# HeyWeCome/WhisprRec

Hardware: AMD Instinct MI355X
Metric: BPR training triplets/sec (higher is better)
Workload: dtype f32; 1 GPU; BPRMF emb_size=64, synthetic 1000000 users x 1000000 items (uniform ids), batch 65536, SGD l2=0, plan build in timed region; batch=65536, emb_size=64, optimizer=SGD, plan_chunk_batches=64, tables=single GPU, step_stream=whisprrec_amd.hip_ops.PipelinedSgd, plan=group plan (no per-batch sort: flags + lists of the shared rows, wr_group.hip), chained_step_launch=True, plan_build=on a side stream, beside the steps of the chunk before

## Files before the change

### whisprrec_amd/csrc/wr_group.hip

```cpp
#include "wr_common.h"
#include <hip/hip_ext.h>

#include <algorithm>

namespace wr {

constexpr int kGpThreads = 1024;
constexpr unsigned kGpRangeBits = 18;
constexpr int kGpWords = 1 << (kGpRangeBits - 5);
constexpr int kGpCap = 8192;
constexpr int kGpBins = 4096;
constexpr int kGpMaxBin = 256;
constexpr int kGpMaxRanges = 8;
constexpr int64_t kGpMaxBatch = 1 << 17;
constexpr int kGpLongRun = 64;
constexpr int kGpMetaWords = 16;
#ifndef WR_GP_DBG
#define WR_GP_DBG 0
#endif

struct GroupLayout {
    int64_t nb, B, fw;
    int R_u, R_i, cap_u, cap_i;
    unsigned mask_u, mask_i, hbits_u, hbits_i;
    int64_t flags, ucnt, icnt, ul_row, ul_src, il_row, il_src, total;
    int64_t zero_words;
};

static inline int ranges_for(int64_t n_rows, unsigned *mask, unsigned *hbits, int *cap) {
    unsigned bits = kGpRangeBits;
    while (bits < kGpRangeBits + 3 && (int64_t(1) << bits) < n_rows) ++bits;
    *mask = (1u << bits) - 1u;
    *hbits = bits;
    const int R = 1 << (bits - kGpRangeBits);
    *cap = kGpCap;
    return R;
}

static bool group_layout(int64_t n, int64_t B, int64_t n_users, int64_t n_items, GroupLayout &L) {
    if (n <= 0 || n >= (int64_t(1) << 31) || B <= 0 || B > kGpMaxBatch) return false;
    if (n_users <= 0 || n_users >= (int64_t(1) << 31) || n_items <= 0 || n_items >= (int64_t(1) << 31)) return false;
    L.nb = (n + B - 1) / B;
    L.B = B;
    L.fw = (B + 31) / 32;
    L.R_u = ranges_for(n_users, &L.mask_u, &L.hbits_u, &L.cap_u);
    L.R_i = ranges_for(n_items, &L.mask_i, &L.hbits_i, &L.cap_i);
    L.flags = kGpMetaWords;
    L.ucnt = L.flags + L.nb * L.fw * 4;
    L.icnt = L.ucnt + align_up(L.nb * L.R_u, 4);
    L.zero_words = L.icnt + align_up(L.nb * L.R_i, 4);
    L.ul_row = L.zero_words;
    L.ul_src = L.ul_row + L.nb * L.R_u * (int64_t)L.cap_u;
    L.il_row = L.ul_src + L.nb * L.R_u * (int64_t)L.cap_u;
    L.il_src = L.il_row + L.nb * L.R_i * (int64_t)L.cap_i;
    L.total = L.il_src + L.nb * L.R_i * (int64_t)L.cap_i;
    return true;
}

struct GpDev {
    int *meta;
    unsigned *flags;
    int *ucnt, *icnt;
    int *ul_row, *ul_src, *il_row, *il_src;
    int R_u, R_i, cap_u, cap_i;
    unsigned mask_u, mask_i, hbits_u, hbits_i;
    int fw;
};

static inline GpDev group_dev(int32_t *plan, const GroupLayout &L) {
    return GpDev{plan, reinterpret_cast<unsigned *>(plan + L.flags), plan + L.ucnt, plan + L.icnt, plan + L.ul_row,
                 plan + L.ul_src, plan + L.il_row, plan + L.il_src, L.R_u, L.R_i, L.cap_u, L.cap_i, L.mask_u, L.mask_i,
                 L.hbits_u, L.hbits_i, (int)L.fw};
}

template <typename F>
__device__ __forceinline__ void gp_scan(const int *__restrict__ a, int cnt, F f) {
    if ((reinterpret_cast<uintptr_t>(a) & 15u) == 0) {
        const int n4 = cnt >> 2;
        const int4 *a4 = reinterpret_cast<const int4 *>(a);
        int i = threadIdx.x;
        for (; i + 3 * kGpThreads < n4; i += 4 * kGpThreads) {
            int4 v[4];
#pragma unroll
            for (int q = 0; q < 4; ++q) v[q] = a4[i + q * kGpThreads];
#pragma unroll
            for (int q = 0; q < 4; ++q) {
                const int at = 4 * (i + q * kGpThreads);
                f(v[q].x, at);
                f(v[q].y, at + 1);
                f(v[q].z, at + 2);
                f(v[q].w, at + 3);
            }
        }
        for (; i < n4; i += kGpThreads) {
            const int4 v = a4[i];
            f(v.x, 4 * i);
            f(v.y, 4 * i + 1);
            f(v.z, 4 * i + 2);
            f(v.w, 4 * i + 3);
        }
        for (int j = (n4 << 2) + threadIdx.x; j < cnt; j += kGpThreads) f(a[j], j);
    } else {
        for (int j = threadIdx.x; j < cnt; j += kGpThreads) f(a[j], j);
    }
}

__global__ __launch_bounds__(kGpThreads) void group_plan_kernel(const int *__restrict__ u, const int *__restrict__ p,
                                                                 const int *__restrict__ n, int64_t n_total, int B, int nb,
                                                                 int n_users, int n_items, GpDev L) {
    extern __shared__ __attribute__((aligned(16))) unsigned gp_lds[];
    unsigned *seen = gp_lds;
    unsigned long long *keys = reinterpret_cast<unsigned long long *>(gp_lds);
    unsigned *multi = gp_lds + 2 * kGpCap;
    unsigned *f0 = multi + kGpWords, *f1 = f0 + L.fw, *f2 = f1 + L.fw;
    int &n_list = *reinterpret_cast<int *>(f2 + L.fw);
    const int per = L.R_u + L.R_i;
    const unsigned lb = xcd_contiguous_id(blockIdx.x, gridDim.x);
    const int b = (int)(lb / (unsigned)per), rr = (int)(lb % (unsigned)per);
    const bool item = rr >= L.R_u;
    const unsigned r = (unsigned)(item ? rr - L.R_u : rr);
    const int64_t base = (int64_t)b * B;
    const int Bb = (int)((base + B <= n_total) ? B : (n_total - base));
    const unsigned n_rows = (unsigned)(item ? n_items : n_users);
    const unsigned mask = item ? L.mask_i : L.mask_u;
    const unsigned rb = (item ? L.hbits_i : L.hbits_u) - kGpRangeBits, rsel = (1u << rb) - 1u;
    for (int i = threadIdx.x; i < kGpWords; i += kGpThreads) {
        seen[i] = 0u;
        multi[i] = 0u;
    }
    for (int i = threadIdx.x; i < 3 * L.fw; i += kGpThreads) f0[i] = 0u;
    if (threadIdx.x == 0) n_list = 0;
    __syncthreads();
    auto mark = [&](int row, int) {
        if ((unsigned)row >= n_rows) {
            L.meta[0] = 1;
            return;
        }
        const unsigned h = (unsigned)row & mask;
        if ((h & rsel) != r) return;
        const unsigned bit = h >> rb, m = 1u << (bit & 31u);
        const unsigned old = atomicOr(&seen[bit >> 5], m);
        if (old & m) atomicOr(&multi[bit >> 5], m);
    };
    if (!(WR_GP_DBG & 8)) {
        if (item) {
            gp_scan(p + base, Bb, mark);
            gp_scan(n + base, Bb, mark);
        } else {
            gp_scan(u + base, Bb, mark);
        }
    }
    __syncthreads();
    auto several = [&](int row) -> bool {
        const unsigned h = (unsigned)row & mask;
        if ((h & rsel) != r) return false;
        const unsigned bit = h >> rb;
        return (multi[bit >> 5] >> (bit & 31u)) & 1u;
    };
    auto append = [&](int row, unsigned src) {
        const int pos = atomicAdd(&n_list, 1);
        if (pos < kGpCap) keys[pos] = ((unsigned long long)(unsigned)row << 32) | src;
    };
    if (!(WR_GP_DBG & 2)) {
        const bool next = b + 1 < nb && !(WR_GP_DBG & 16);
        const int64_t nbase = base + B;
        const int Bn = next ? (int)((nbase + B <= n_total) ? B : (n_total - nbase)) : 0;
        auto defer = [&](int row, int t) {
            if (several(row)) atomicOr(&f2[t >> 5], 1u << (t & 31));
        };
        if (item) {
            gp_scan(p + base, Bb, [&](int row, int t) {
                if (several(row)) {
                    atomicOr(&f0[t >> 5], 1u << (t & 31));
                    append(row, (unsigned)t << 1);
                }
            });
            gp_scan(n + base, Bb, [&](int row, int t) {
                if (several(row)) {
                    atomicOr(&f1[t >> 5], 1u << (t & 31));
                    append(row, ((unsigned)t << 1) | 1u);
                }
            });
            gp_scan(p + nbase, Bn, defer);
            gp_scan(n + nbase, Bn, defer);
        } else {
            gp_scan(u + base, Bb, [&](int row, int t) {
                if (several(row)) {
                    atomicOr(&f0[t >> 5], 1u << (t & 31));
                    append(row, (unsigned)t << 1);
                }
            });
            gp_scan(u + nbase, Bn, defer);
        }
    }
    __syncthreads();
    if (!(WR_GP_DBG & 4)) {
        unsigned *fb = L.flags + (int64_t)b * L.fw * 4;
        for (int w = threadIdx.x; w < L.fw; w += kGpThreads) {
            if (f0[w]) __hip_atomic_fetch_or(fb + 4 * w + (item ? 1 : 0), f0[w], __ATOMIC_RELAXED, __HIP_MEMORY_SCOPE_AGENT);
            if (item && f1[w]) __hip_atomic_fetch_or(fb + 4 * w + 2, f1[w], __ATOMIC_RELAXED, __HIP_MEMORY_SCOPE_AGENT);
            if (f2[w])
                __hip_atomic_fetch_or(fb + 4 * (L.fw + w) + 3, f2[w], __ATOMIC_RELAXED, __HIP_MEMORY_SCOPE_AGENT);
        }
    }
    const int cap = item ? L.cap_i : L.cap_u, R = item ? L.R_i : L.R_u;
    int m = n_list;
    if (m > cap) {
        if (threadIdx.x == 0) L.meta[1] = 1;
        m = cap;
    }
    int *cnt = reinterpret_cast<int *>(multi);
    unsigned short *out16 = reinterpret_cast<unsigned short *>(multi + kGpBins);
    int *wave_tot = reinterpret_cast<int *>(f0);
    auto bin_of = [&](unsigned long long k) -> int { return (int)(((((unsigned)(k >> 32)) & mask) >> rb) & (kGpBins - 1)); };
    int *lrow = (item ? L.il_row : L.ul_row) + ((int64_t)b * R + r) * cap, *lsrc = (item ? L.il_src : L.ul_src) + ((int64_t)b * R + r) * cap;
    __syncthreads();
    for (int i = threadIdx.x; i < kGpBins; i += kGpThreads) cnt[i] = 0;
    __syncthreads();
    if (!(WR_GP_DBG & 1)) {
        for (int j = threadIdx.x; j < m; j += kGpThreads) atomicAdd(&cnt[bin_of(keys[j])], 1);
        __syncthreads();
        constexpr int kOwn = kGpBins / kGpThreads;
        const int c0 = (int)threadIdx.x * kOwn;
        int local = 0;
#pragma unroll
        for (int j = 0; j < kOwn; ++j) local += cnt[c0 + j];
        int incl = local;
#pragma unroll
        for (int d = 1; d < 64; d <<= 1) {
            const int v = __shfl_up(incl, d, 64);
            if ((int)(threadIdx.x & 63) >= d) incl += v;
        }
        if ((threadIdx.x & 63) == 63) wave_tot[threadIdx.x >> 6] = incl;
        __syncthreads();
        int run = incl - local;
        for (int w = 0; w < (int)(threadIdx.x >> 6); ++w) run += wave_tot[w];
#pragma unroll
        for (int j = 0; j < kOwn; ++j) {
            const int c = cnt[c0 + j];
            cnt[c0 + j] = run;
            run += c;
        }
        __syncthreads();
        for (int j = threadIdx.x; j < m; j += kGpThreads) out16[atomicAdd(&cnt[bin_of(keys[j])], 1)] = (unsigned short)j;
        __syncthreads();
        for (int j = threadIdx.x; j < m; j += kGpThreads) {
            const unsigned long long k = keys[j];
            const int bin = bin_of(k);
            const int lo = bin ? cnt[bin - 1] : 0, hi = cnt[bin];
            if (hi - lo > kGpMaxBin) {
                L.meta[1] = 1;
                continue;
            }
            int pos = lo, same = 0;
            for (int jj = lo; jj < hi; ++jj) {
                const unsigned long long o = keys[out16[jj]];
                pos += o < k ? 1 : 0;
                same += (unsigned)(o >> 32) == (unsigned)(k >> 32) ? 1 : 0;
            }
            if (same > kGpLongRun) L.meta[2] = 1;
            lrow[pos] = (int)(k >> 32);
            lsrc[pos] = (int)(unsigned)k;
        }
    } else {
        for (int j = threadIdx.x; j < m; j += kGpThreads) {
            lrow[j] = (int)(keys[j] >> 32);
            lsrc[j] = (int)(unsigned)keys[j];
        }
    }
    if (threadIdx.x == 0) (item ? L.icnt : L.ucnt)[(int64_t)b * R + r] = m;
}

__global__ __launch_bounds__(kBlock) void narrow_ids_kernel(const int64_t *__restrict__ u, const int64_t *__restrict__ p,
                                                             const int64_t *__restrict__ n, int *__restrict__ u32,
                                                             int *__restrict__ p32, int *__restrict__ n32, int64_t cnt) {
    const int64_t i = (int64_t)blockIdx.x * kBlock + threadIdx.x;
    if (i >= cnt) return;
    const int64_t a = u[i], b = p[i], c = n[i];
    u32[i] = (a >= 0 && a < (int64_t(1) << 31)) ? (int)a : -1;
    p32[i] = (b >= 0 && b < (int64_t(1) << 31)) ? (int)b : -1;
    n32[i] = (c >= 0 && c < (int64_t(1) << 31)) ? (int)c : -1;
}

constexpr int kGsTile = 32;
constexpr int kGsAhead = 8;
constexpr int kGsShards = 64;
constexpr int kGsShardStride = 16;
constexpr int kGsStepWords = kGsShards * kGsShardStride;
constexpr int kGsDefChunk = 32;
constexpr int kGsLdsInts = 1024 + 8;
constexpr unsigned kGsSpinLimit = 1u << 22;

struct GsBatch {
    const int *u, *p, *n;
    const uint4 *flags;
    const int *ul_row, *ul_src, *ul_cnt, *il_row, *il_src, *il_cnt;
    int B, R_u, R_i, cap_u, cap_i;
};

struct GsArgs {
    float *U, *I;
    int D;
    float lr;
    GsBatch cur;
    float *Z, *ZU, *partials;
    float denom;
    GsBatch prev;
    const float *Zp, *ZUp, *partials_prev;
    int n_partials_prev;
    float denom_prev;
    float *loss_prev;
    int nA, nIT, nUT, nDS, tiles_at, side_at;
    int chained;
    unsigned *done, *timeout;
    float *Gs;
    int nL;
};

template <int NV>
__device__ __forceinline__ Row<NV> row_zero() {
    Row<NV> r;
#pragma unroll
    for (int k = 0; k < NV; ++k) r.v[k] = make_float4(0.f, 0.f, 0.f, 0.f);
    return r;
}

template <int T, int NV, bool FULL>
__device__ __forceinline__ void gs_single(const GsArgs &a, int t, int u, int p, int n, bool us, bool ps, bool ns, int lane,
                                          float &terms) {
    const Row<NV> ur = load_row<T, NV, FULL>(a.U, u, a.D, lane);
    const Row<NV> pr = load_row<T, NV, FULL>(a.I, p, a.D, lane);
    const Row<NV> nr = load_row<T, NV, FULL>(a.I, n, a.D, lane);
    const float sp = team_sum<T>(dot_partial<NV>(ur, pr));
    const float sn = team_sum<T>(dot_partial<NV>(ur, nr));
    float term, c;
    bpr_terms(sp, sn, a.denom, term, c);
    terms += term;
    Row<NV> g, z;
#pragma unroll
    for (int k = 0; k < NV; ++k) {
        g.v[k] = make_float4(c * (pr.v[k].x - nr.v[k].x), c * (pr.v[k].y - nr.v[k].y), c * (pr.v[k].z - nr.v[k].z),
                             c * (pr.v[k].w - nr.v[k].w));
        z.v[k] = make_float4(c * ur.v[k].x, c * ur.v[k].y, c * ur.v[k].z, c * ur.v[k].w);
    }
    const float lr = a.lr;
    if (!us) {
        Row<NV> w;
#pragma unroll
        for (int k = 0; k < NV; ++k)
            w.v[k] = make_float4(ur.v[k].x - lr * g.v[k].x, ur.v[k].y - lr * g.v[k].y, ur.v[k].z - lr * g.v[k].z,
                                 ur.v[k].w - lr * g.v[k].w);
        store_row<T, NV, FULL>(a.U, u, a.D, lane, w);
    } else {
        store_row<T, NV, FULL>(a.ZU, t, a.D, lane, g);
// ... 410 lines not shown
            a.denom_prev = global_batch > 0 ? (float)global_batch : (float)a.prev.B;
            a.loss_prev = at_or_null(g.loss_out, k - 1);
            a.nIT = (int)std::min<int64_t>(WR_GS_NIT, (2 * B + kGsTile - 1) / kGsTile + L.R_i);
            a.nUT = (int)std::min<int64_t>(WR_GS_NUT, (B + kGsTile - 1) / kGsTile + L.R_u);
        }
        a.tiles_at = (int)((int64_t)a.nA * WR_GS_TILES_AT / 16);
        a.side_at = std::max(a.tiles_at, (int)((int64_t)a.nA * WR_GS_SIDE_AT / 16));
        const dim3 grid((unsigned)(a.nA + a.nIT + a.nUT + a.nDS));
        hipEvent_t e0 = have_cur ? ev(k, 0) : nullptr, e1 = have_cur ? ev(k, 1) : nullptr;
        if (e0 != nullptr || e1 != nullptr)
            hipExtLaunchKernelGGL((bprmf_group_step<T, NV, FULL>), grid, dim3(kBlock), 0, g.stream, e0, e1, 0, a);
        else
            hipLaunchKernelGGL((bprmf_group_step<T, NV, FULL>), grid, dim3(kBlock), 0, g.stream, a);
        WR_LAUNCH_CHECK("bprmf_group_step");
        n_partials_prev = a.nA + a.nDS;
    }
    return WR_OK;
}

static int32_t check_group_plan(const char *entry, const GroupRun &g, GroupLayout &L) {
    int32_t rc;
    if ((rc = check_whole_lines(entry, whole_lines(g.tabs.U, g.tabs.I, g.tabs.D), g.tabs.D)) != WR_OK) return rc;
    WR_REQUIRE(group_layout(g.n_triplets, g.batch_size, g.tabs.n_users, g.tabs.n_items, L), WR_E_RANGE,
               "group plan not applicable to n=%lld, batch=%lld", (long long)g.n_triplets, (long long)g.batch_size);
    WR_REQUIRE(g.plan_words >= L.total, WR_E_WORKSPACE, "group plan: %lld words < %lld", (long long)g.plan_words, (long long)L.total);
    return WR_OK;
}

static int32_t run_group(const char *entry, GroupRun &g, const GroupLayout &L, int64_t sync_batches) {
    int32_t rc;
    if ((rc = check_workspace(entry, g.workspace, g.workspace_bytes, 2 * gs_ws_one(g.batch_size, g.tabs.D))) != WR_OK) return rc;
    if ((rc = check_sync_words(entry, g.sync, g.sync_words, sync_batches * kGsStepWords + 4)) != WR_OK) return rc;
    if (g.range.n_batches == 0) return WR_OK;
    if (g.n_cu == 0 && (rc = device_cu_count(&g.n_cu)) != WR_OK) return rc;
    const GpDev G = group_dev(const_cast<int32_t *>(g.plan), L);
#define WR_CALL_GS(T_, NV_, FULL_) return launch_group_steps<T_, NV_, FULL_>(g, L, G)
    WR_DISPATCH_D(g.tabs.D, WR_CALL_GS);
#undef WR_CALL_GS
    return WR_OK;
}

}

using namespace wr;

extern "C" {

int64_t wr_group_plan_words(int64_t n_triplets, int64_t batch_size, int64_t n_users, int64_t n_items) {
    GroupLayout L;
    if (!group_layout(n_triplets, batch_size, n_users, n_items, L)) return 0;
    return L.total;
}

int32_t wr_group_plan_layout(int64_t n_triplets, int64_t batch_size, int64_t n_users, int64_t n_items, int64_t *out) {
    WR_REQUIRE(out != nullptr, WR_E_NULL, "out is NULL");
    GroupLayout L;
    WR_REQUIRE(group_layout(n_triplets, batch_size, n_users, n_items, L), WR_E_RANGE,
               "group plan not applicable to n=%lld, batch=%lld", (long long)n_triplets, (long long)batch_size);
    const int64_t v[16] = {L.nb, L.fw, L.R_u, L.R_i, (int64_t)L.mask_u, (int64_t)L.mask_i, L.flags, L.ucnt, L.icnt, L.ul_row,
                           L.ul_src, L.il_row, L.il_src, L.total, L.cap_u, L.cap_i};
    for (int i = 0; i < 16; ++i) out[i] = v[i];
    return WR_OK;
}

int32_t wr_narrow_ids_i64(const int64_t *u, const int64_t *p, const int64_t *n, int32_t *u32, int32_t *p32, int32_t *n32,
                          int64_t count, void *stream_) {
    WR_REQUIRE(u && p && n && u32 && p32 && n32, WR_E_NULL, "index arrays must not be NULL");
    WR_REQUIRE(count >= 0 && count < (int64_t(1) << 40), WR_E_SHAPE, "count out of range");
    if (count == 0) return WR_OK;
    hipLaunchKernelGGL(narrow_ids_kernel, dim3((unsigned)((count + kBlock - 1) / kBlock)), dim3(kBlock), 0,
                       reinterpret_cast<hipStream_t>(stream_), u, p, n, u32, p32, n32, count);
    WR_LAUNCH_CHECK("narrow_ids_kernel");
    return WR_OK;
}

int32_t wr_group_plan_build(const int32_t *u, const int32_t *p, const int32_t *n, int64_t n_triplets, int64_t batch_size,
                            int64_t n_users, int64_t n_items, int32_t *plan, int64_t plan_words, void *stream_) {
    WR_REQUIRE(u && p && n && plan, WR_E_NULL, "index arrays / plan must not be NULL");
    GroupLayout L;
    WR_REQUIRE(group_layout(n_triplets, batch_size, n_users, n_items, L), WR_E_RANGE,
               "group plan not applicable to n=%lld, batch=%lld", (long long)n_triplets, (long long)batch_size);
    WR_REQUIRE(aligned16(plan) && plan_words >= L.total, WR_E_WORKSPACE, "group plan: %lld words < %lld", (long long)plan_words,
               (long long)L.total);
    WR_REQUIRE(L.nb * (L.R_u + L.R_i) < (int64_t(1) << 31), WR_E_SHAPE, "group plan: too many batches in one plan");
    hipStream_t stream = reinterpret_cast<hipStream_t>(stream_);
    WR_HIP(hipMemsetAsync(plan, 0, (size_t)L.zero_words * 4, stream));
    const size_t lds = (size_t)(2 * kGpCap + kGpWords + 3 * L.fw + 4) * 4;
    static bool attr_set = false;
    if (!attr_set) {
        WR_HIP(hipFuncSetAttribute(reinterpret_cast<const void *>(group_plan_kernel), hipFuncAttributeMaxDynamicSharedMemorySize,
                                   (int)((2 * kGpCap + kGpWords + 3 * ((kGpMaxBatch + 31) / 32) + 4) * 4)));
        attr_set = true;
    }
    const GpDev G = group_dev(plan, L);
    hipLaunchKernelGGL(group_plan_kernel, dim3((unsigned)(L.nb * (L.R_u + L.R_i))), dim3(kGpThreads), lds, stream, u, p, n,
                       n_triplets, (int)batch_size, (int)L.nb, (int)n_users, (int)n_items, G);
    WR_LAUNCH_CHECK("group_plan_kernel");
    return WR_OK;
}

int64_t wr_bprmf_group_workspace_bytes(int64_t batch_size, int32_t D) { return 2 * gs_ws_one(batch_size, D); }

int64_t wr_bprmf_group_sync_words(int64_t n_batches) { return n_batches < 0 ? WR_E_SHAPE : (n_batches + 1) * kGsStepWords + 4; }

int32_t wr_bprmf_group_supported(const float *user_tab, const float *item_tab, int32_t D) {
    return (user_tab && item_tab && D >= 4 && D <= 1024 && D % 4 == 0 && whole_lines(user_tab, item_tab, D)) ? 1 : 0;
}

int32_t wr_bprmf_run_sgd_group(float *user_tab, int64_t n_users, float *item_tab, int64_t n_items, int32_t D,
                               const int32_t *u, const int32_t *p, const int32_t *n, int64_t n_triplets, int64_t batch_size,
                               const int32_t *plan, int64_t plan_words, int64_t first_batch, int64_t n_batches, float lr,
                               float *loss_out, void *const *events, void *workspace, int64_t workspace_bytes, int32_t *sync,
                               int64_t sync_words, void *stream) {
    GroupRun g{};
    g.tabs = TablePair{user_tab, item_tab, n_users, n_items, D};
    g.u = u; g.p = p; g.n = n; g.n_triplets = n_triplets; g.batch_size = batch_size;
    g.plan = plan; g.plan_words = plan_words;
    g.range = BatchRange{first_batch, n_batches};
    g.lr = lr; g.loss_out = loss_out; g.events = events;
    g.workspace = workspace; g.workspace_bytes = workspace_bytes;
    g.sync = reinterpret_cast<uint32_t *>(sync); g.sync_words = sync_words;
    g.stream = reinterpret_cast<hipStream_t>(stream);
    int32_t rc;
    GroupLayout L;
    if ((rc = check_tables(g.tabs)) != WR_OK) return rc;
    WR_REQUIRE(u && p && n && plan && sync, WR_E_NULL, "index arrays / plan / sync words must not be NULL");
    if ((rc = check_group_plan("wr_bprmf_run_sgd_group", g, L)) != WR_OK) return rc;
    WR_REQUIRE(first_batch >= 0 && n_batches >= 0 && first_batch + n_batches <= L.nb, WR_E_SHAPE,
               "batches [%lld,%lld) exceed the plan's %lld", (long long)first_batch, (long long)(first_batch + n_batches),
               (long long)L.nb);
    return run_group("wr_bprmf_run_sgd_group", g, L, n_batches + 1);
}

int32_t wr_bprmf_shard_step_group(float *user_shard, int64_t n_user_rows, float *item_ext, int64_t n_ext_rows,
                                  int64_t n_local_items, int32_t D, const int32_t *vu, const int32_t *vp, const int32_t *vn,
                                  int64_t n_triplets, int64_t batch_size, const int32_t *plan, int64_t plan_words, int64_t batch,
                                  int64_t global_batch, float lr, float *grad_slots, float *loss_partial, void *workspace,
                                  int64_t workspace_bytes, int32_t *sync, int64_t sync_words, void *stream) {
    GroupRun g{};
    g.tabs = TablePair{user_shard, item_ext, n_user_rows, n_ext_rows, D};
    g.u = vu; g.p = vp; g.n = vn; g.n_triplets = n_triplets; g.batch_size = batch_size;
    g.plan = plan; g.plan_words = plan_words;
    g.range = BatchRange{batch, 1};
    g.lr = lr; g.loss_out = loss_partial;
    g.workspace = workspace; g.workspace_bytes = workspace_bytes;
    g.sync = reinterpret_cast<uint32_t *>(sync); g.sync_words = sync_words;
    g.n_cu = 256;
    g.grad_slots = grad_slots; g.n_local_items = n_local_items; g.global_batch = global_batch;
    g.stream = reinterpret_cast<hipStream_t>(stream);
    int32_t rc;
    GroupLayout L;
    if ((rc = check_tables(g.tabs, "user_shard", "item_ext")) != WR_OK) return rc;
    WR_REQUIRE(vu && vp && vn && plan && sync && grad_slots, WR_E_NULL, "index arrays / plan / sync words / grad_slots must not be NULL");
    WR_REQUIRE(aligned16(grad_slots), WR_E_ALIGN, "grad_slots is not 16-byte aligned");
    WR_REQUIRE(n_local_items >= 0 && n_local_items <= n_ext_rows, WR_E_SHAPE, "n_local_items %lld outside [0, %lld]",
               (long long)n_local_items, (long long)n_ext_rows);
    if ((rc = check_group_plan("wr_bprmf_shard_step_group", g, L)) != WR_OK) return rc;
    WR_REQUIRE(batch >= 0 && batch < L.nb, WR_E_SHAPE, "batch %lld outside the plan's %lld", (long long)batch, (long long)L.nb);
    WR_REQUIRE(global_batch >= batch_size, WR_E_SHAPE, "global_batch %lld < local batch %lld", (long long)global_batch,
               (long long)batch_size);
    return run_group("wr_bprmf_shard_step_group", g, L, 2);
}

}
```

### whisprrec_amd/hip_ops.py

```python
import ctypes

import torch

from . import abi


def _stream():
    return torch.cuda.current_stream().cuda_stream


def _p(t):
    return None if t is None else t.data_ptr()


def _addr(struct):
    return ctypes.addressof(struct) if struct is not None else None


def _event_handles(events, per_step, count, allow_none):
    if events is None:
        return None
    if len(events) != per_step * count:
        raise ValueError("%s must hold %d events per step" % ("phase_events" if per_step == 4 else "events", per_step))
    handles = []
# ... 1574 lines not shown
        use_group = self.group and runner is None and len(live) == 1 and first >= 2 and \
            self.GROUP_MIN_BATCH <= B <= 131072 and u_all.dtype in (torch.int32, torch.int64) and \
            min_rows >= self.GROUP_MIN_ROWS_PER_TRIPLET * B and \
            all(sg["tabs"].group_supported() for sg in segs if sg["tabs"] is not None)
        garenas = self._garena_pair(U.device, B, first, U.shape[0], n_items) if use_group else None
        arenas = None if use_group else self._arena_pair(U.device, B, first, n_items if use_chain else 0)
        for a in (arenas or []) + (garenas or []):
            a.release_after(main)
        h = {"segs": segs, "B": B, "u": u_all, "p": p_all, "n": n_all, "nb": first, "n_users": U.shape[0], "n_items": n_items,
             "at": 0, "tag": 0, "next": None, "cur": None, "map": None, "arenas": arenas, "pos": 0,
             "group": use_group, "garenas": garenas, "device": U.device,
             "ids32": [torch.empty(u_all.numel(), dtype=torch.int32, device=U.device) for _ in range(3)]
                      if use_group and u_all.dtype == torch.int64 else None,
             "chain": use_chain, "prep": prep, "runner": runner, "inline": bool(self.inline_plan),
             "lead": [int(c) for c in (first_chunk if isinstance(first_chunk, (list, tuple)) else [first_chunk or 0]) if c]}
        self.plan_stream.wait_stream(main)
        self._prefetch(h)
        return h

    def _build_stream(self, h):
        return torch.cuda.current_stream(h["u"].device) if h["inline"] else self.plan_stream

    def _prefetch(self, h):
        if h["at"] >= h["nb"]:
            h["next"] = None
            return
        first, B = h["at"], h["B"]
        c = min(self.chunk_batches(B), h["nb"] - first)
        if h["lead"]:
            c = min(c, h["lead"].pop(0))
        h["at"] += c
        lo, hi = first * B, min(h["u"].numel(), (first + c) * B)
        with torch.cuda.stream(self._build_stream(h)):
            bmap = h["map"] if h["map"] else None
            if h["prep"] is not None:
                h["prep"].fill(lo, hi)
            if h["group"]:
                cols = (h["u"], h["p"], h["n"])
                if h["ids32"] is not None:
                    abi.check(abi.lib().wr_narrow_ids_i64(*[_p(c[lo:hi]) for c in cols], *[_p(c[lo:hi]) for c in h["ids32"]],
                                                          hi - lo, _stream()), "wr_narrow_ids_i64")
                    cols = h["ids32"]
                plan = self.ops.GroupPlan(cols[0][lo:hi], cols[1][lo:hi], cols[2][lo:hi], B, h["n_users"], h["n_items"],
                                          arena=h["garenas"][h["tag"]], defer=True)
                h["tag"] ^= 1
                h["next"] = (first, plan)
                return
            if h["arenas"] is None:
                h["arenas"] = self._arena_pair(h["device"], B, h["nb"], h["n_items"] if h["chain"] else 0)
            plan = self.ops.BatchPlan(h["u"][lo:hi], h["p"][lo:hi], h["n"][lo:hi], B, h["n_users"], h["n_items"],
                                      validate=False, ws_tag="rot%d" % h["tag"], bucket_map=bmap, arena=h["arenas"][h["tag"]],
                                      defer=True, overlap=h["chain"])
        h["tag"] ^= 1
        h["next"] = (first, plan)

    STICKY_MSG = "a wait inside a step launch expired (hand-off between the workgroups of one launch): the tables are not " \
                 "valid — do not save or evaluate them; restart the run"

    def _queue_sticky(self, h, tabs, main):
        words = tabs.sticky_words()
        if not words:
            return
        pin = h.get("sticky_pin")
        if pin is None or pin.numel() < 2 * len(words):
            pin = h["sticky_pin"] = torch.zeros(2 * max(len(words), 4), dtype=torch.int32, pin_memory=True)
        half = pin.numel() // 2
        off = half * (h.get("sticky_tag", 0) & 1)
        h["sticky_tag"] = h.get("sticky_tag", 0) + 1
        for j, wd in enumerate(words):
            pin[off + j:off + j + 1].copy_(wd, non_blocking=True)
        ev = torch.cuda.Event()
        ev.record(main)
        self._check_sticky(h)
        h["sticky_pending"] = (ev, pin[off:off + len(words)])

    def _check_sticky(self, h):
        pend = h.pop("sticky_pending", None)
        if pend is not None:
            pend[0].synchronize()
            if bool(pend[1].numpy().any()):
                raise abi.WhisprRecHipError(self.STICKY_MSG)

    def _take_next(self, h, pos, main):
        self._check_sticky(h)
        if h["next"] is None:
            self._prefetch(h)
        cur = h["next"]
        assert cur is not None and cur[0] == pos, "steps must be run in order"
        plan = cur[1]
        plan.validate()
        if isinstance(plan, GroupPlan):
            if plan.overflow or plan.long_run:
                h["group"] = False
                self.stats["group_fallbacks"] += 1
                if h["next"] is not None and h["next"][0] != cur[0]:
                    raise AssertionError("plan pipeline out of step")
                if plan.overflow:
                    first, B = cur[0], h["B"]
                    lo, hi = first * B, first * B + plan.n_triplets
                    plan.arena.release_after(main)
                    if h["arenas"] is None:
                        h["arenas"] = self._arena_pair(h["device"], B, h["nb"], h["n_items"] if h["chain"] else 0)
                    with torch.cuda.stream(self._build_stream(h)):
                        plan = self.ops.BatchPlan(h["u"][lo:hi], h["p"][lo:hi], h["n"][lo:hi], B, h["n_users"], h["n_items"],
                                                  validate=False, ws_tag="rot%d" % h["tag"], arena=h["arenas"][h["tag"]],
                                                  defer=True, overlap=h["chain"])
                    h["tag"] ^= 1
                    plan.validate()
                    cur = (first, plan)
            main.wait_event(plan.ready)
            h["cur"], h["next"] = cur, None
            return cur
        main.wait_event(plan.ready)
        if plan.fast_overflowed:
            if plan._mapped():
                h["map"] = False
            elif h["map"] is None:
                with torch.cuda.stream(self._build_stream(h)):
                    src = (h["prep"].users, h["prep"].items) if h["prep"] is not None else (h["u"], h["p"])
                    h["map"] = self.ops.BucketMap(src[0], src[1], h["n_users"], h["n_items"], h["B"])
        if h["chain"] and plan.hot is not None:
            h["chain"] = False
        if h["chain"] and plan.hot is None and plan.overlap is not None and not plan.overlap["fits"]:
            dcn = plan.overlap["def_count_np"]
            if int((dcn[1:] > plan.overlap["cap"]).sum()) * 2 > plan.n_batches - 1:
                h["chain"] = False
        h["cur"], h["next"] = cur, None
        return cur

    def _run_span(self, h, sg, pos, end, lr, losses, loss_off):
        main = torch.cuda.current_stream(sg["tabs"].U.device)
        while pos < end:
            cur = h["cur"]
            if cur is None or pos >= cur[0] + cur[1].n_batches:
                cur = self._take_next(h, pos, main)
            base, plan = cur
            c = min(end, base + plan.n_batches) - pos
            if h["inline"] and h["next"] is None and h["at"] < h["nb"]:
                mid = base + plan.n_batches // 2
                if pos >= mid:
                    self._prefetch(h)
                else:
                    c = min(c, mid - pos)
            elif self.PREFETCH_AFTER_TRIPLETS > 0 and h["next"] is None and h["at"] < h["nb"] and \
                    c > (self.PREFETCH_AFTER_TRIPLETS + h["B"] - 1) // h["B"]:
                c = (self.PREFETCH_AFTER_TRIPLETS + h["B"] - 1) // h["B"]
            if isinstance(plan, GroupPlan):
                sg["tabs"].run_sgd_group(plan, pos - base, c, lr, losses=losses[loss_off:loss_off + c])
                self.stats["group_calls"] += 1
            elif h["runner"] is not None:
                h["runner"](plan, pos - base, c, losses[loss_off:loss_off + c])
                self.stats["plain_calls"] += 1
            elif h["chain"] and plan.overlap is not None and c >= 2:
                sg["tabs"].run_sgd_chain(plan, pos - base, c, lr, losses=losses[loss_off:loss_off + c])
                self.stats["chain_calls"] += 1
            else:
                sg["tabs"].run_sgd(plan, pos - base, c, lr, losses=losses[loss_off:loss_off + c])
                self.stats["plain_calls"] += 1
            pos += c
            loss_off += c
            if pos >= base + plan.n_batches:
                plan.arena.release_after(main)
                self._queue_sticky(h, sg["tabs"], main)
            if h["next"] is None and not h["inline"]:
                self._prefetch(h)
        h["pos"] = pos

# ... 645 lines not shown
```

Measured before the change: 2.573 billion triplets/s.

## Merge group-plan ranges into wide super-ranges with scratch-list duplicate detection

The group plan kernel now has each block cover a super-range of up to 2^20 rows instead of one 2^18-row range, which cuts the number of blocks that each rescan the same batch ids. Duplicates are found in one pass: first-seen bits go into an LDS bitmap and repeats are written to a scratch list in global memory, which then rebuilds the multi bitmap. The scan helper now separates a cheap predicate from the action, collecting hit bits so that only hits do the expensive work. Per-range sorting runs sequentially inside the block, and a per-step sticky-error check is dropped from the Python path, which removes a possible host synchronization but delays error detection.

Measured after the change: 2.637 billion triplets/s (median of 6 runs). +2.5%, better.

```diff
diff --git a/whisprrec_amd/csrc/wr_group.hip b/whisprrec_amd/csrc/wr_group.hip
--- a/whisprrec_amd/csrc/wr_group.hip
+++ b/whisprrec_amd/csrc/wr_group.hip
@@ -5,9 +5,13 @@
 
 namespace wr {
 
+#ifndef WR_GP_WIDE_BITS
+#define WR_GP_WIDE_BITS 20
+#endif
+
 constexpr int kGpThreads = 1024;
 constexpr unsigned kGpRangeBits = 18;
-constexpr int kGpWords = 1 << (kGpRangeBits - 5);
+constexpr unsigned kGpWideBits = WR_GP_WIDE_BITS;
 constexpr int kGpCap = 8192;
 constexpr int kGpBins = 4096;
 constexpr int kGpMaxBin = 256;
@@ -15,6 +19,10 @@
 constexpr int64_t kGpMaxBatch = 1 << 17;
 constexpr int kGpLongRun = 64;
 constexpr int kGpMetaWords = 16;
+constexpr int kGpLdsBytes = 163840;
+constexpr int kGpOrderWords = 2 * kGpCap + kGpBins + kGpCap / 2;
+constexpr int kGpTailWords = 32;
+static_assert(kGpWideBits >= kGpRangeBits && kGpWideBits <= kGpRangeBits + 3, "a super-range is a union of ranges");
 #ifndef WR_GP_DBG
 #define WR_GP_DBG 0
 #endif
@@ -23,9 +31,20 @@
     int64_t nb, B, fw;
     int R_u, R_i, cap_u, cap_i;
     unsigned mask_u, mask_i, hbits_u, hbits_i;
+    unsigned sbits_u, sbits_i;
     int64_t flags, ucnt, icnt, ul_row, ul_src, il_row, il_src, total;
     int64_t zero_words;
 };
+
+static inline int64_t gp_lds_words(unsigned sbits, int64_t fw) {
+    return std::max<int64_t>(int64_t(1) << (sbits - 5), kGpOrderWords) + 3 * fw + kGpTailWords;
+}
+
+static inline unsigned super_bits(unsigned hbits, int64_t fw) {
+    unsigned s = std::min(hbits, kGpWideBits);
+    while (s > kGpRangeBits && gp_lds_words(s, fw) * 4 > kGpLdsBytes) --s;
+    return s;
+}
 
 static inline int ranges_for(int64_t n_rows, unsigned *mask, unsigned *hbits, int *cap) {
     unsigned bits = kGpRangeBits;
@@ -45,6 +64,8 @@
     L.fw = (B + 31) / 32;
     L.R_u = ranges_for(n_users, &L.mask_u, &L.hbits_u, &L.cap_u);
     L.R_i = ranges_for(n_items, &L.mask_i, &L.hbits_i, &L.cap_i);
+    L.sbits_u = super_bits(L.hbits_u, L.fw);
+    L.sbits_i = super_bits(L.hbits_i, L.fw);
     L.flags = kGpMetaWords;
     L.ucnt = L.flags + L.nb * L.fw * 4;
     L.icnt = L.ucnt + align_up(L.nb * L.R_u, 4);
@@ -65,43 +86,55 @@
     int R_u, R_i, cap_u, cap_i;
     unsigned mask_u, mask_i, hbits_u, hbits_i;
     int fw;
+    unsigned sbits_u, sbits_i;
 };
 
 static inline GpDev group_dev(int32_t *plan, const GroupLayout &L) {
     return GpDev{plan, reinterpret_cast<unsigned *>(plan + L.flags), plan + L.ucnt, plan + L.icnt, plan + L.ul_row,
                  plan + L.ul_src, plan + L.il_row, plan + L.il_src, L.R_u, L.R_i, L.cap_u, L.cap_i, L.mask_u, L.mask_i,
-                 L.hbits_u, L.hbits_i, (int)L.fw};
-}
-
-template <typename F>
-__device__ __forceinline__ void gp_scan(const int *__restrict__ a, int cnt, F f) {
+                 L.hbits_u, L.hbits_i, (int)L.fw, L.sbits_u, L.sbits_i};
+}
+
+#ifndef WR_GP_AHEAD
+#define WR_GP_AHEAD 4
+#endif
+
+template <typename F1, typename F2>
+__device__ __forceinline__ void gp_scan(const int *__restrict__ a, int cnt, F1 look, F2 act) {
     if ((reinterpret_cast<uintptr_t>(a) & 15u) == 0) {
+        constexpr int kA = WR_GP_AHEAD;
         const int n4 = cnt >> 2;
         const int4 *a4 = reinterpret_cast<const int4 *>(a);
         int i = threadIdx.x;
-        for (; i + 3 * kGpThreads < n4; i += 4 * kGpThreads) {
-            int4 v[4];
-#pragma unroll
-            for (int q = 0; q < 4; ++q) v[q] = a4[i + q * kGpThreads];
-#pragma unroll
-            for (int q = 0; q < 4; ++q) {
-                const int at = 4 * (i + q * kGpThreads);
-                f(v[q].x, at);
-                f(v[q].y, at + 1);
-                f(v[q].z, at + 2);
-                f(v[q].w, at + 3);
+        for (; i + (kA - 1) * kGpThreads < n4; i += kA * kGpThreads) {
+            int4 v[kA];
+            unsigned hits = 0u;
+#pragma unroll
+            for (int q = 0; q < kA; ++q) v[q] = a4[i + q * kGpThreads];
+#pragma unroll
+            for (int q = 0; q < kA; ++q)
+                hits |= (look(v[q].x) << (4 * q)) | (look(v[q].y) << (4 * q + 1)) | (look(v[q].z) << (4 * q + 2)) |
+                        (look(v[q].w) << (4 * q + 3));
+            while (hits) {
+                const int k = __ffs(hits) - 1;
+                hits &= hits - 1u;
+                const int at = 4 * (i + (k >> 2) * kGpThreads) + (k & 3);
+                act(a[at], at);
             }
         }
         for (; i < n4; i += kGpThreads) {
             const int4 v = a4[i];
-            f(v.x, 4 * i);
-            f(v.y, 4 * i + 1);
-            f(v.z, 4 * i + 2);
-            f(v.w, 4 * i + 3);
-        }
-        for (int j = (n4 << 2) + threadIdx.x; j < cnt; j += kGpThreads) f(a[j], j);
+            const unsigned t0 = look(v.x), t1 = look(v.y), t2 = look(v.z), t3 = look(v.w);
+            if (t0) act(v.x, 4 * i);
+            if (t1) act(v.y, 4 * i + 1);
+            if (t2) act(v.z, 4 * i + 2);
+            if (t3) act(v.w, 4 * i + 3);
+        }
+        for (int j = (n4 << 2) + threadIdx.x; j < cnt; j += kGpThreads)
+            if (look(a[j])) act(a[j], j);
     } else {
-        for (int j = threadIdx.x; j < cnt; j += kGpThreads) f(a[j], j);
+        for (int j = threadIdx.x; j < cnt; j += kGpThreads)
+            if (look(a[j])) act(a[j], j);
     }
 }
 
@@ -109,88 +142,106 @@
                                                                  const int *__restrict__ n, int64_t n_total, int B, int nb,
                                                                  int n_users, int n_items, GpDev L) {
     extern __shared__ __attribute__((aligned(16))) unsigned gp_lds[];
-    unsigned *seen = gp_lds;
-    unsigned long long *keys = reinterpret_cast<unsigned long long *>(gp_lds);
-    unsigned *multi = gp_lds + 2 * kGpCap;
-    unsigned *f0 = multi + kGpWords, *f1 = f0 + L.fw, *f2 = f1 + L.fw;
-    int &n_list = *reinterpret_cast<int *>(f2 + L.fw);
-    const int per = L.R_u + L.R_i;
+    const unsigned G_u = 1u << (L.hbits_u - L.sbits_u), G_i = 1u << (L.hbits_i - L.sbits_i), per = G_u + G_i;
     const unsigned lb = xcd_contiguous_id(blockIdx.x, gridDim.x);
-    const int b = (int)(lb / (unsigned)per), rr = (int)(lb % (unsigned)per);
-    const bool item = rr >= L.R_u;
-    const unsigned r = (unsigned)(item ? rr - L.R_u : rr);
+    const int b = (int)(lb / per);
+    const unsigned rr = lb % per;
+    const bool item = rr < G_i;
+    const unsigned g = item ? rr : rr - G_i;
     const int64_t base = (int64_t)b * B;
     const int Bb = (int)((base + B <= n_total) ? B : (n_total - base));
     const unsigned n_rows = (unsigned)(item ? n_items : n_users);
-    const unsigned mask = item ? L.mask_i : L.mask_u;
-    const unsigned rb = (item ? L.hbits_i : L.hbits_u) - kGpRangeBits, rsel = (1u << rb) - 1u;
-    for (int i = threadIdx.x; i < kGpWords; i += kGpThreads) {
-        seen[i] = 0u;
-        multi[i] = 0u;
-    }
-    for (int i = threadIdx.x; i < 3 * L.fw; i += kGpThreads) f0[i] = 0u;
-    if (threadIdx.x == 0) n_list = 0;
+    const unsigned mask = item ? L.mask_i : L.mask_u, hbits = item ? L.hbits_i : L.hbits_u, sbits = item ? L.sbits_i : L.sbits_u;
+    const unsigned lg = hbits - sbits, gsel = (1u << lg) - 1u;
+    const unsigned rb = hbits - kGpRangeBits, ls = rb - lg;
+    const int R = 1 << rb, S = 1 << ls;
+    const int cap = item ? L.cap_i : L.cap_u;
+    const int bm_words = 1 << (sbits - 5);
+    const int region = bm_words > kGpOrderWords ? bm_words : kGpOrderWords;
+    unsigned *bm = gp_lds;
+    unsigned *f0 = gp_lds + region, *f1 = f0 + L.fw, *f2 = f1 + L.fw;
+    int *seg_cnt = reinterpret_cast<int *>(f2 + L.fw);
+    int &n_scr = seg_cnt[kGpMaxRanges];
+    int *wave_tot = seg_cnt + 16;
+    int *lrow_b = (item ? L.il_row : L.ul_row) + ((int64_t)b * R + g) * cap, *lsrc_b = (item ? L.il_src : L.ul_src) + ((int64_t)b * R + g) * cap;
+    const int64_t seg_stride = (int64_t)cap << lg;
+    for (int i = threadIdx.x; i < bm_words; i += kGpThreads) bm[i] = 0u;
+    for (int i = threadIdx.x; i < 3 * L.fw + kGpTailWords; i += kGpThreads) f0[i] = 0u;
     __syncthreads();
+    const int scr_cap = cap << ls;
+    auto see = [&](int row) -> unsigned {
+        const unsigned h = (unsigned)row & mask, bit = h >> lg;
+        const bool bad = (unsigned)row >= n_rows;
+        const unsigned m = (!bad && (h & gsel) == g) ? 1u << (bit & 31u) : 0u;
+        const unsigned old = atomicOr(&bm[bit >> 5], m);
+        return ((old & m) != 0u || bad) ? 1u : 0u;
+    };
     auto mark = [&](int row, int) {
         if ((unsigned)row >= n_rows) {
             L.meta[0] = 1;
             return;
         }
-        const unsigned h = (unsigned)row & mask;
-        if ((h & rsel) != r) return;
-        const unsigned bit = h >> rb, m = 1u << (bit & 31u);
-        const unsigned old = atomicOr(&seen[bit >> 5], m);
-        if (old & m) atomicOr(&multi[bit >> 5], m);
+        const int q = atomicAdd(&n_scr, 1);
+        if (q < scr_cap) lrow_b[(int64_t)(q & (S - 1)) * seg_stride + (q >> ls)] = (int)(((unsigned)row & mask) >> lg);
     };
     if (!(WR_GP_DBG & 8)) {
         if (item) {
-            gp_scan(p + base, Bb, mark);
-            gp_scan(n + base, Bb, mark);
+            gp_scan(p + base, Bb, see, mark);
+            gp_scan(n + base, Bb, see, mark);
         } else {
-            gp_scan(u + base, Bb, mark);
+            gp_scan(u + base, Bb, see, mark);
         }
     }
     __syncthreads();
-    auto several = [&](int row) -> bool {
-        const unsigned h = (unsigned)row & mask;
-        if ((h & rsel) != r) return false;
-        const unsigned bit = h >> rb;
-        return (multi[bit >> 5] >> (bit & 31u)) & 1u;
+    int n_s = n_scr;
+    if (n_s > scr_cap) {
+        if (threadIdx.x == 0) L.meta[1] = 1;
+        n_s = scr_cap;
+    }
+    for (int i = threadIdx.x; i < bm_words; i += kGpThreads) bm[i] = 0u;
+    __syncthreads();
+    if (!(WR_GP_DBG & 32)) {
+        for (int q = threadIdx.x; q < n_s; q += kGpThreads) {
+            const unsigned bit = (unsigned)lrow_b[(int64_t)(q & (S - 1)) * seg_stride + (q >> ls)] & ((1u << sbits) - 1u);
+            atomicOr(&bm[bit >> 5], 1u << (bit & 31u));
+        }
+    }
+    __syncthreads();
+    auto several = [&](int row) -> unsigned {
+        const unsigned h = (unsigned)row & mask, bit = h >> lg;
+        const unsigned w = bm[bit >> 5];
+        return (h & gsel) == g ? (w >> (bit & 31u)) & 1u : 0u;
     };
     auto append = [&](int row, unsigned src) {
-        const int pos = atomicAdd(&n_list, 1);
-        if (pos < kGpCap) keys[pos] = ((unsigned long long)(unsigned)row << 32) | src;
+        const int j = (int)((((unsigned)row & mask) >> lg) & (unsigned)(S - 1));
+        const int pos = atomicAdd(&seg_cnt[j], 1);
+        if (pos < cap) {
+            lrow_b[j * seg_stride + pos] = row;
+            lsrc_b[j * seg_stride + pos] = (int)src;
+        }
     };
     if (!(WR_GP_DBG & 2)) {
         const bool next = b + 1 < nb && !(WR_GP_DBG & 16);
         const int64_t nbase = base + B;
         const int Bn = next ? (int)((nbase + B <= n_total) ? B : (n_total - nbase)) : 0;
-        auto defer = [&](int row, int t) {
-            if (several(row)) atomicOr(&f2[t >> 5], 1u << (t & 31));
-        };
+        auto defer = [&](int, int t) { atomicOr(&f2[t >> 5], 1u << (t & 31)); };
         if (item) {
-            gp_scan(p + base, Bb, [&](int row, int t) {
-                if (several(row)) {
-                    atomicOr(&f0[t >> 5], 1u << (t & 31));
-                    append(row, (unsigned)t << 1);
-                }
+            gp_scan(p + base, Bb, several, [&](int row, int t) {
+                atomicOr(&f0[t >> 5], 1u << (t & 31));
+                append(row, (unsigned)t << 1);
             });
-            gp_scan(n + base, Bb, [&](int row, int t) {
-                if (several(row)) {
-                    atomicOr(&f1[t >> 5], 1u << (t & 31));
-                    append(row, ((unsigned)t << 1) | 1u);
-                }
+            gp_scan(n + base, Bb, several, [&](int row, int t) {
+                atomicOr(&f1[t >> 5], 1u << (t & 31));
+                append(row, ((unsigned)t << 1) | 1u);
             });
-            gp_scan(p + nbase, Bn, defer);
-            gp_scan(n + nbase, Bn, defer);
+            gp_scan(p + nbase, Bn, several, defer);
+            gp_scan(n + nbase, Bn, several, defer);
         } else {
-            gp_scan(u + base, Bb, [&](int row, int t) {
-                if (several(row)) {
-                    atomicOr(&f0[t >> 5], 1u << (t & 31));
-                    append(row, (unsigned)t << 1);
-                }
+            gp_scan(u + base, Bb, several, [&](int row, int t) {
+                atomicOr(&f0[t >> 5], 1u << (t & 31));
+                append(row, (unsigned)t << 1);
             });
-            gp_scan(u + nbase, Bn, defer);
+            gp_scan(u + nbase, Bn, several, defer);
         }
     }
     __syncthreads();
@@ -203,73 +254,87 @@
                 __hip_atomic_fetch_or(fb + 4 * (L.fw + w) + 3, f2[w], __ATOMIC_RELAXED, __HIP_MEMORY_SCOPE_AGENT);
         }
     }
-    const int cap = item ? L.cap_i : L.cap_u, R = item ? L.R_i : L.R_u;
-    int m = n_list;
-    if (m > cap) {
-        if (threadIdx.x == 0) L.meta[1] = 1;
-        m = cap;
-    }
-    int *cnt = reinterpret_cast<int *>(multi);
-    unsigned short *out16 = reinterpret_cast<unsigned short *>(multi + kGpBins);
-    int *wave_tot = reinterpret_cast<int *>(f0);
+    unsigned long long *keys = reinterpret_cast<unsigned long long *>(gp_lds);
+    int *cnt = reinterpret_cast<int *>(gp_lds + 2 * kGpCap);
+    unsigned short *out16 = reinterpret_cast<unsigned short *>(gp_lds + 2 * kGpCap + kGpBins);
     auto bin_of = [&](unsigned long long k) -> int { return (int)(((((unsigned)(k >> 32)) & mask) >> rb) & (kGpBins - 1)); };
-    int *lrow = (item ? L.il_row : L.ul_row) + ((int64_t)b * R + r) * cap, *lsrc = (item ? L.il_src : L.ul_src) + ((int64_t)b * R + r) * cap;
-    __syncthreads();
-    for (int i = threadIdx.x; i < kGpBins; i += kGpThreads) cnt[i] = 0;
-    __syncthreads();
-    if (!(WR_GP_DBG & 1)) {
-        for (int j = threadIdx.x; j < m; j += kGpThreads) atomicAdd(&cnt[bin_of(keys[j])], 1);
+    for (int j = 0; j < S; ++j) {
+        int *lrow = lrow_b + j * seg_stride, *lsrc = lsrc_b + j * seg_stride;
         __syncthreads();
-        constexpr int kOwn = kGpBins / kGpThreads;
-        const int c0 = (int)threadIdx.x * kOwn;
-        int local = 0;
-#pragma unroll
-        for (int j = 0; j < kOwn; ++j) local += cnt[c0 + j];
-        int incl = local;
-#pragma unroll
-        for (int d = 1; d < 64; d <<= 1) {
-            const int v = __shfl_up(incl, d, 64);
-            if ((int)(threadIdx.x & 63) >= d) incl += v;
-        }
-        if ((threadIdx.x & 63) == 63) wave_tot[threadIdx.x >> 6] = incl;
-        __syncthreads();
-        int run = incl - local;
-        for (int w = 0; w < (int)(threadIdx.x >> 6); ++w) run += wave_tot[w];
-#pragma unroll
-        for (int j = 0; j < kOwn; ++j) {
-            const int c = cnt[c0 + j];
-            cnt[c0 + j] = run;
-            run += c;
-        }
-        __syncthreads();
-        for (int j = threadIdx.x; j < m; j += kGpThreads) out16[atomicAdd(&cnt[bin_of(keys[j])], 1)] = (unsigned short)j;
-        __syncthreads();
-        for (int j = threadIdx.x; j < m; j += kGpThreads) {
-            const unsigned long long k = keys[j];
-            const int bin = bin_of(k);
-            const int lo = bin ? cnt[bin - 1] : 0, hi = cnt[bin];
-            if (hi - lo > kGpMaxBin) {
-                L.meta[1] = 1;
-                continue;
-            }
-            int pos = lo, same = 0;
-            for (int jj = lo; jj < hi; ++jj) {
-                const unsigned long long o = keys[out16[jj]];
-                pos += o < k ? 1 : 0;
-                same += (unsigned)(o >> 32) == (unsigned)(k >> 32) ? 1 : 0;
-            }
-            if (same > kGpLongRun) L.meta[2] = 1;
-            lrow[pos] = (int)(k >> 32);
-            lsrc[pos] = (int)(unsigned)k;
-        }
-    } else {
-        for (int j = threadIdx.x; j < m; j += kGpThreads) {
-            lrow[j] = (int)(keys[j] >> 32);
-            lsrc[j] = (int)(unsigned)keys[j];
-        }
-    }
-    if (threadIdx.x == 0) (item ? L.icnt : L.ucnt)[(int64_t)b * R + r] = m;
-}
+        int m = seg_cnt[j];
+        if (m > cap) {
+            if (threadIdx.x == 0) L.meta[1] = 1;
+            m = cap;
+        }
+        if (!(WR_GP_DBG & 1)) {
+            {
+                constexpr int kMine = kGpCap / kGpThreads;
+                int kr[kMine], ks[kMine];
+#pragma unroll
+                for (int q = 0; q < kMine; ++q) {
+                    const int i = (int)threadIdx.x + q * kGpThreads, ic = i < m ? i : 0;
+                    kr[q] = lrow[ic];
+                    ks[q] = lsrc[ic];
+                }
+#pragma unroll
+                for (int q = 0; q < kMine; ++q) {
+                    const int i = (int)threadIdx.x + q * kGpThreads;
+                    if (i < m) keys[i] = ((unsigned long long)(unsigned)kr[q] << 32) | (unsigned)ks[q];
+                }
+            }
+            for (int i = threadIdx.x; i < kGpBins; i += kGpThreads) cnt[i] = 0;
+            __syncthreads();
+            for (int i = threadIdx.x; i < m; i += kGpThreads) atomicAdd(&cnt[bin_of(keys[i])], 1);
+            __syncthreads();
+            constexpr int kOwn = kGpBins / kGpThreads;
+            const int c0 = (int)threadIdx.x * kOwn;
+            int local = 0;
+#pragma unroll
+            for (int i = 0; i < kOwn; ++i) local += cnt[c0 + i];
+            int incl = local;
+#pragma unroll
+            for (int d = 1; d < 64; d <<= 1) {
+                const int v = __shfl_up(incl, d, 64);
+                if ((int)(threadIdx.x & 63) >= d) incl += v;
+            }
+            if ((threadIdx.x & 63) == 63) wave_tot[threadIdx.x >> 6] = incl;
+            __syncthreads();
+            int run = incl - local;
+            for (int w = 0; w < (int)(threadIdx.x >> 6); ++w) run += wave_tot[w];
+#pragma unroll
+            for (int i = 0; i < kOwn; ++i) {
+                const int c = cnt[c0 + i];
+                cnt[c0 + i] = run;
+                run += c;
+            }
+            __syncthreads();
+            for (int i = threadIdx.x; i < m; i += kGpThreads) out16[atomicAdd(&cnt[bin_of(keys[i])], 1)] = (unsigned short)i;
+            __syncthreads();
+            for (int i = threadIdx.x; i < m; i += kGpThreads) {
+                const unsigned long long k = keys[i];
+                const int bin = bin_of(k);
+                const int lo = bin ? cnt[bin - 1] : 0, hi = cnt[bin];
+                if (hi - lo > kGpMaxBin) {
+                    L.meta[1] = 1;
+                    continue;
+                }
+                int pos = lo, same = 0;
+                for (int jj = lo; jj < hi; ++jj) {
+                    const unsigned long long o = keys[out16[jj]];
+                    pos += o < k ? 1 : 0;
+                    same += (unsigned)(o >> 32) == (unsigned)(k >> 32) ? 1 : 0;
+                }
+                if (same > kGpLongRun) L.meta[2] = 1;
+                lrow[pos] = (int)(k >> 32);
+                lsrc[pos] = (int)(unsigned)k;
+            }
+        }
+        const int used = n_s > j ? (n_s - j + S - 1) >> ls : 0;
+        for (int i = m + (int)threadIdx.x; i < used; i += kGpThreads) lrow[i] = 0;
+        if (threadIdx.x == 0) (item ? L.icnt : L.ucnt)[(int64_t)b * R + g + ((int64_t)j << lg)] = m;
+    }
+}
+
 
 __global__ __launch_bounds__(kBlock) void narrow_ids_kernel(const int64_t *__restrict__ u, const int64_t *__restrict__ p,
                                                              const int64_t *__restrict__ n, int *__restrict__ u32,
@@ -846,18 +911,20 @@
                "group plan not applicable to n=%lld, batch=%lld", (long long)n_triplets, (long long)batch_size);
     WR_REQUIRE(aligned16(plan) && plan_words >= L.total, WR_E_WORKSPACE, "group plan: %lld words < %lld", (long long)plan_words,
                (long long)L.total);
-    WR_REQUIRE(L.nb * (L.R_u + L.R_i) < (int64_t(1) << 31), WR_E_SHAPE, "group plan: too many batches in one plan");
+    const int64_t per = (int64_t(1) << (L.hbits_u - L.sbits_u)) + (int64_t(1) << (L.hbits_i - L.sbits_i));
+    WR_REQUIRE(L.nb * per < (int64_t(1) << 31), WR_E_SHAPE, "group plan: too many batches in one plan");
     hipStream_t stream = reinterpret_cast<hipStream_t>(stream_);
     WR_HIP(hipMemsetAsync(plan, 0, (size_t)L.zero_words * 4, stream));
-    const size_t lds = (size_t)(2 * kGpCap + kGpWords + 3 * L.fw + 4) * 4;
+    const size_t lds = (size_t)std::max(gp_lds_words(L.sbits_u, L.fw), gp_lds_words(L.sbits_i, L.fw)) * 4;
+    WR_REQUIRE(lds <= (size_t)kGpLdsBytes, WR_E_SHAPE, "group plan: %lld bytes of LDS", (long long)lds);
     static bool attr_set = false;
     if (!attr_set) {
         WR_HIP(hipFuncSetAttribute(reinterpret_cast<const void *>(group_plan_kernel), hipFuncAttributeMaxDynamicSharedMemorySize,
-                                   (int)((2 * kGpCap + kGpWords + 3 * ((kGpMaxBatch + 31) / 32) + 4) * 4)));
+                                   kGpLdsBytes));
         attr_set = true;
     }
     const GpDev G = group_dev(plan, L);
-    hipLaunchKernelGGL(group_plan_kernel, dim3((unsigned)(L.nb * (L.R_u + L.R_i))), dim3(kGpThreads), lds, stream, u, p, n,
+    hipLaunchKernelGGL(group_plan_kernel, dim3((unsigned)(L.nb * per)), dim3(kGpThreads), lds, stream, u, p, n,
                        n_triplets, (int)batch_size, (int)L.nb, (int)n_users, (int)n_items, G);
     WR_LAUNCH_CHECK("group_plan_kernel");
     return WR_OK;
diff --git a/whisprrec_amd/hip_ops.py b/whisprrec_amd/hip_ops.py
--- a/whisprrec_amd/hip_ops.py
+++ b/whisprrec_amd/hip_ops.py
@@ -1680,7 +1680,6 @@
                 raise abi.WhisprRecHipError(self.STICKY_MSG)
 
     def _take_next(self, h, pos, main):
-        self._check_sticky(h)
         if h["next"] is None:
             self._prefetch(h)
         cur = h["next"]
```
